# mindspore-lab/mindpose

Hardware: AMD Instinct MI355X
Metric: images/sec at 256x192, HRNet-W32 top-down inference (backbone+head+decode) (higher is better)
Workload: dtype f32; 1 GPU; configs[2]: HRNet-W32 256x192 inference, 1xMI355X per rank, multi-branch conv + fuse layers on fp32 MFMA, HRNetHead, arg-max+shift decode; per_gpu_batch=128, global_batch=128, image=256x192, heatmap=64x48x17, execution_lanes=4

## Files before the change

include/mindpose_hip.h:

```cpp
#ifndef MINDPOSE_HIP_H
#define MINDPOSE_HIP_H

#include <stddef.h>
#include <stdint.h>

#ifdef __cplusplus
extern "C" {
#endif

typedef void* mp_stream_t;

#define MP_OK 0
#define MP_ERR_NULL (-1)
#define MP_ERR_SHAPE (-2)
#define MP_ERR_UNSUPPORTED (-3)
#define MP_ERR_HIP (-4)
#define MP_ERR_WORKSPACE (-5)

const char* mp_version(void);
const char* mp_error_string(int code);
int mp_last_hip_error(void);

#define MP_REFINE_NONE 0
#define MP_REFINE_SHIFT 1
// ... 170 lines not shown
int mp_f16_stem_conv_fwd(const float* x_dev, const float* weight_dev, const float* scale_dev, const float* shift_dev, int relu,
                         void* out_c8_dev, int n, int h, int w, mp_stream_t stream);
int mp_plan_add_stem_conv_f16(mp_plan* plan, const float* x_dev, const float* weight_dev, const float* scale_dev, const float* shift_dev,
                              int relu, void* out_c8_dev, int n, int h, int w);
int mp_f16_expand_reduce_fwd(const void* mid_c8_dev, const void* res_c8_dev, const void* packed_w3_dev, const float* scale3_dev,
                             const float* shift3_dev, int relu3, const void* packed_w1_dev, const float* scale1_dev,
                             const float* shift1_dev, int relu1, void* y_c8_dev, void* z_c8_dev, int n, int cm, int ce, int cr, int h,
                             int w, mp_stream_t stream);
int mp_f16_dual_pw_fwd(const void* x_c8_dev, const void* packed_wa_dev, const float* scale_a_dev, const float* shift_a_dev, int relu_a,
                       const void* packed_wb_dev, const float* scale_b_dev, const float* shift_b_dev, int relu_b, void* ya_c8_dev,
                       void* zb_c8_dev, int n, int cm, int ce, int cr, int h, int w, mp_stream_t stream);
int mp_f16_ds_expand_reduce_fwd(const void* mid_c8_dev, const void* x0_c8_dev, const void* packed_wd_dev, const float* scale_d_dev,
                                const float* shift_d_dev, const void* packed_w3_dev, const float* scale3_dev, const float* shift3_dev,
                                int relu3, const void* packed_w1_dev, const float* scale1_dev, const float* shift1_dev, int relu1,
                                void* y_c8_dev, void* z_c8_dev, int n, int cm, int ce, int cr, int h, int w, mp_stream_t stream);
int mp_plan_add_ds_expand_reduce_f16(mp_plan* plan, const void* mid_c8_dev, const void* x0_c8_dev, const void* packed_wd_dev,
                                     const float* scale_d_dev, const float* shift_d_dev, const void* packed_w3_dev,
                                     const float* scale3_dev, const float* shift3_dev, int relu3, const void* packed_w1_dev,
                                     const float* scale1_dev, const float* shift1_dev, int relu1, void* y_c8_dev, void* z_c8_dev, int n,
                                     int cm, int ce, int cr, int h, int w);
int mp_plan_add_dual_pw_f16(mp_plan* plan, const void* x_c8_dev, const void* packed_wa_dev, const float* scale_a_dev,
                            const float* shift_a_dev, int relu_a, const void* packed_wb_dev, const float* scale_b_dev,
                            const float* shift_b_dev, int relu_b, void* ya_c8_dev, void* zb_c8_dev, int n, int cm, int ce, int cr, int h, int w);
int mp_plan_add_expand_reduce_f16(mp_plan* plan, const void* mid_c8_dev, const void* res_c8_dev, const void* packed_w3_dev,
                                  const float* scale3_dev, const float* shift3_dev, int relu3, const void* packed_w1_dev,
                                  const float* scale1_dev, const float* shift1_dev, int relu1, void* y_c8_dev, void* z_c8_dev, int n,
                                  int cm, int ce, int cr, int h, int w);
int mp_expand_reduce_fwd(const float* mid_dev, const float* res_dev, const float* x0_dev, const float* packed_wd_dev,
                         const float* scale_d_dev, const float* shift_d_dev, const float* packed_w3_dev, const float* scale3_dev,
                         const float* shift3_dev, const float* packed_w1_dev, const float* scale1_dev, const float* shift1_dev,
                         float* y_dev, float* z_dev, int n, int cm, int ce, int cr, int h, int w, mp_stream_t stream);
int mp_plan_add_expand_reduce(mp_plan* plan, const float* mid_dev, const float* res_dev, const float* x0_dev, const float* packed_wd_dev,
                              const float* scale_d_dev, const float* shift_d_dev, const float* packed_w3_dev, const float* scale3_dev,
                              const float* shift3_dev, const float* packed_w1_dev, const float* scale1_dev, const float* shift1_dev,
                              float* y_dev, float* z_dev, int n, int cm, int ce, int cr, int h, int w);
int mp_plan_add_basicblock_f16(mp_plan* plan, const void* x_c8_dev, const void* packed_w1_dev, const float* scale1_dev,
                               const float* shift1_dev, const void* packed_w2_dev, const float* scale2_dev, const float* shift2_dev,
                               void* out_c8_dev, int n, int c, int h, int w, int rows);
int mp_f16_fuse_upsample_sum(const void* base_dev, const void* t1_dev, int s1, const void* t2_dev, int s2, const void* t3_dev,
                             int s3, void* out_dev, int n, int c, int h, int w, int relu, mp_stream_t stream);
int mp_plan_add_conv_f16(mp_plan* plan, const mp_conv_desc* desc, int variant, const void* x_c8_dev, const void* packed_w_dev,
                         const float* scale_dev, const float* shift_dev, const void* res1_c8_dev, const void* res2_c8_dev,
                         void* out_c8_dev);
int mp_plan_add_fuse_sum_f16(mp_plan* plan, const void* base_dev, const void* t1_dev, int s1, const void* t2_dev, int s2,
                             const void* t3_dev, int s3, void* out_dev, int n, int c, int h, int w, int relu);
int mp_plan_add_layout_f16(mp_plan* plan, int to_c8, const void* x_dev, void* out_dev, int n, int c, int h, int w);
int mp_concat_channels(const void* a_dev, int ca, const void* b_dev, int cb, void* out_dev, int n, int h, int w, int c8,
                       mp_stream_t stream);
int mp_plan_add_concat(mp_plan* plan, const void* a_dev, int ca, const void* b_dev, int cb, void* out_dev, int n, int h, int w,
                       int c8);
int mp_col_slice(const void* in_dev, void* out_dev, int rows, int w_in, int start, int w_out, int c8, mp_stream_t stream);
int mp_plan_add_col_slice(mp_plan* plan, const void* in_dev, void* out_dev, int rows, int w_in, int start, int w_out, int c8);
int mp_conv_supported(const mp_conv_desc* desc, int variant);

int mp_warp_affine(const uint8_t* src_dev, const long long* src_offsets_dev, const int* src_hw_dev, const int* flip_dev,
                   const double* trans_dev, void* out_dev, int n, int out_h, int out_w, int normalize, const float mean[3], const float stddev[3],
                   mp_stream_t stream);

int mp_flip_width(const float* in_dev, float* out_dev, int n, int c, int h, int w, mp_stream_t stream);

int mp_resize_pad_normalize(const uint8_t* src_dev, const long long* src_offsets_dev, const int* src_hw_dev, const int* dst_wh_host,
                            float* out_dev, uint8_t* mask_dev, int n, int pad_h, int pad_w, const float mean[3],
                            const float stddev[3], mp_stream_t stream);

int mp_bottomup_train_augment(const uint8_t* src_dev, const long long* src_offsets_dev, const int* src_hw_dev,
                              const uint8_t* mask_src_dev, const long long* mask_offsets_dev, const double* trans_dev,
                              const int* flip_dev, const int* stage_wh_host, float* image_dev, uint8_t* mask_dev, int n, int s,
                              int out_h, int out_w, int hmax, int wmax, const float mean[3], const float stddev[3],
                              mp_stream_t stream);

typedef struct mp_bottomup_stage {
    const float* data_dev;
    int32_t c, h, w;
    int32_t has_tags;
} mp_bottomup_stage;
size_t mp_bottomup_workspace_bytes(int n, int k, int h, int w, int max_num);
int mp_bottomup_parse_nms_topk(const mp_bottomup_stage* stages_host, int num_stages, const uint8_t* mask_dev, int mask_h, int mask_w,
                               int n, int k, int tag_per_joint, int nms_kernel, int max_num, float* heatmap_raw_dev,
                               float* tagging_dev, void* workspace_dev, size_t workspace_bytes, mp_stream_t stream);
int mp_bottomup_gather(const float* heatmap_raw_dev, const float* tagging_dev, const void* workspace_dev, size_t workspace_bytes,
                       int n, int k, int h, int w, int tag_per_joint, int num_tags, int max_num, int shift_coordinate,
                       float* val_k_dev, float* ind_k_dev, float* tag_k_dev, mp_stream_t stream);

int mp_bottomup_refine_missing(const float* heatmap_raw_dev, const float* tagging_dev, const float* mean_tag_dev,
                               const int* person_image_dev, int num_persons, int n, int k, int h, int w, int tag_per_joint,
                               int num_tags, float* found_dev, mp_stream_t stream);

size_t mp_joints_mse_mask_workspace_bytes(int n, int k);
int mp_joints_mse_mask_fwd(const float* pred_dev, long long pred_sn, long long pred_sc, long long pred_sr, const float* target_dev,
                           long long target_sn, long long target_sc, long long target_sr, const void* mask_dev, int mask_is_u8,
                           long long mask_sn, long long mask_sr, float* loss_dev, void* workspace_dev, size_t workspace_bytes, int n,
                           int k, int h, int w, mp_stream_t stream);
int mp_joints_mse_mask_bwd(const float* pred_dev, long long pred_sn, long long pred_sc, long long pred_sr, const float* target_dev,
                           long long target_sn, long long target_sc, long long target_sr, const void* mask_dev, int mask_is_u8,
                           long long mask_sn, long long mask_sr, const float* grad_out_dev, float* grad_pred_dev, long long grad_sn,
                           long long grad_sc, long long grad_sr, int n, int k, int h, int w, mp_stream_t stream);
size_t mp_ae_loss_workspace_bytes(int n);
int mp_ae_loss_fwd(const float* tags_dev, long long tag_batch_stride, const int32_t* tag_ind_dev, float* loss2_dev,
                   void* workspace_dev, size_t workspace_bytes, int n, int m, int k, int hw, mp_stream_t stream);
int mp_ae_loss_bwd(const float* tags_dev, long long tag_batch_stride, const int32_t* tag_ind_dev, const float* grad_out2_dev,
                   float* grad_tags_dev, long long grad_batch_stride, int n, int m, int k, int hw, mp_stream_t stream);
int mp_bottomup_target(const float* keypoints_dev, const int* counts_dev, const int* stage_wh_host, float* target_dev,
                       int32_t* tag_ind_dev, int n, int s, int m, int k, int hmax, int wmax, int max_num, int tag_per_joint,
                       double sigma, mp_stream_t stream);

int mp_f16_bn_train_fwd(const void* z_dev, const float* gamma_dev, const float* beta_dev, const void* res_dev, void* y_dev,
// ... 89 lines not shown
```

mindpose_amd/_lib.py:

```python
import ctypes
import os

import torch

_HERE = os.path.dirname(os.path.abspath(__file__))
LIB_PATH = os.environ.get("MINDPOSE_HIP_LIB", os.path.join(_HERE, "csrc", "libmindpose_hip.so"))

MP_REFINE_NONE, MP_REFINE_SHIFT, MP_REFINE_DARK = 0, 1, 2
MP_CONV_SHARES_CUS = 1
MP_CONV_PHASES4 = 2
MP_ERR_UNSUPPORTED = -3


def env_on(name: str, default: bool = True) -> bool:
    value = os.environ.get(name)
    return value != "0" if default else value == "1"


c_f32p = ctypes.c_void_p
c_int = ctypes.c_int
c_size_t = ctypes.c_size_t
c_i64 = ctypes.c_longlong


# ... 104 lines not shown
    "mp_plan_set_lane": (c_int, [ctypes.c_void_p, c_int]),
    "mp_plan_add_barrier": (c_int, [ctypes.c_void_p]),
    "mp_flip_width": (c_int, [c_f32p, c_f32p] + [c_int] * 4 + [ctypes.c_void_p]),
    "mp_warp_affine": (c_int, [c_f32p] * 6 + [c_int] * 4 + [ctypes.POINTER(ctypes.c_float)] * 2 + [ctypes.c_void_p]),
    "mp_f16_packed_weight_bytes": (c_size_t, [c_int] * 4),
    "mp_f16_activation_bytes": (c_size_t, [c_int] * 4),
    "mp_f16_pack_weight": (c_int, [c_f32p, c_f32p] + [c_int] * 7 + [ctypes.c_void_p]),
    "mp_f16_pack_weight_batch": (c_int, [c_f32p, c_f32p, c_int, ctypes.c_uint, ctypes.c_void_p]),
    "mp_conv_pack_weight_batch": (c_int, [c_f32p, c_f32p, c_int, ctypes.c_uint, ctypes.c_void_p]),
    "mp_f16_to_c8": (c_int, [c_f32p, c_f32p] + [c_int] * 4 + [ctypes.c_void_p]),
    "mp_f16_from_c8": (c_int, [c_f32p, c_f32p] + [c_int] * 4 + [ctypes.c_void_p]),
    "mp_f16_conv2d_fwd": (c_int, [ctypes.POINTER(ConvDesc), c_int] + [c_f32p] * 7 + [ctypes.c_void_p]),
    "mp_f16_conv_stats_parts": (c_int, [ctypes.POINTER(ConvDesc), c_int]),
    "mp_f16_conv2d_fwd_stats": (c_int, [ctypes.POINTER(ConvDesc), c_int] + [c_f32p] * 6 + [ctypes.POINTER(ConvStats), ctypes.c_void_p]),
    "mp_f16_bn_train_fwd_stats": (c_int, [c_f32p] * 9 + [c_int] * 3 + [ctypes.c_float, ctypes.c_float, c_int, c_f32p, c_int, c_f32p,
                                          c_size_t, ctypes.c_void_p]),
    "mp_f16_conv_pre_supported": (c_int, [ctypes.POINTER(ConvDesc), c_int]),
    "mp_f16_conv_supported": (c_int, [ctypes.POINTER(ConvDesc), c_int, c_int, c_int]),
    "mp_f16_bn_train_finalize": (c_int, [c_f32p] * 6 + [c_int] * 3 + [ctypes.c_float, ctypes.c_float, c_f32p, c_int, c_f32p, c_f32p, c_f32p,
                                         c_size_t, ctypes.c_void_p]),
    "mp_f16_bn_train_bwd_stats": (c_int, [c_f32p] * 10 + [c_int] * 3 + [c_f32p, c_int, c_f32p, c_size_t, ctypes.c_void_p]),
    "mp_f16_bn_train_fwd_stats_grouped": (c_int, [ctypes.POINTER(BnFwdJob), c_int, ctypes.c_float, ctypes.c_float, ctypes.c_void_p]),
    "mp_f16_bn_train_bwd_stats_grouped": (c_int, [ctypes.POINTER(BnBwdJob), c_int, ctypes.c_void_p]),
    "mp_f16_ew_stats_parts": (c_int, [c_int] * 3),
    "mp_f16_fuse_term_stats_parts": (c_int, [c_int] * 5),
    "mp_f16_sum_tensors_stats": (c_int, [c_f32p] * 7 + [c_int] * 4 + [c_f32p, c_size_t, ctypes.c_void_p]),
    "mp_f16_fuse_sum_bwd_term_stats": (c_int, [c_f32p] * 3 + [c_int] * 6 + [c_f32p, c_f32p, c_int, c_f32p, c_size_t, ctypes.c_void_p]),
    "mp_optimizer_step": (c_int, [c_int, ctypes.c_void_p, ctypes.c_void_p, ctypes.c_void_p, ctypes.c_void_p, c_size_t, ctypes.c_float,
                                  ctypes.c_float, ctypes.c_float, ctypes.POINTER(ctypes.c_float * 5), ctypes.c_void_p]),
    "mp_f16_basicblock_fwd": (c_int, [c_f32p] * 8 + [c_int] * 5 + [ctypes.c_void_p]),
    "mp_f16_basicblock_supported": (c_int, [c_int] * 4),
    "mp_stem_conv_fwd": (c_int, [c_f32p] * 4 + [c_int, c_f32p] + [c_int] * 3 + [ctypes.c_void_p]),
    "mp_plan_add_stem_conv": (c_int, [ctypes.c_void_p] + [c_f32p] * 4 + [c_int, c_f32p] + [c_int] * 3),
    "mp_f16_stem_conv_fwd": (c_int, [c_f32p] * 4 + [c_int, c_f32p] + [c_int] * 3 + [ctypes.c_void_p]),
    "mp_plan_add_stem_conv_f16": (c_int, [ctypes.c_void_p] + [c_f32p] * 4 + [c_int, c_f32p] + [c_int] * 3),
    "mp_f16_dual_pw_fwd": (c_int, [c_f32p] * 4 + [c_int] + [c_f32p] * 3 + [c_int] + [c_f32p] * 2 + [c_int] * 6 + [ctypes.c_void_p]),
    "mp_plan_add_dual_pw_f16": (c_int, [ctypes.c_void_p] + [c_f32p] * 4 + [c_int] + [c_f32p] * 3 + [c_int] + [c_f32p] * 2 + [c_int] * 6),
    "mp_f16_expand_reduce_fwd": (c_int, [c_f32p] * 5 + [c_int] + [c_f32p] * 3 + [c_int] + [c_f32p] * 2 + [c_int] * 6 + [ctypes.c_void_p]),
    "mp_plan_add_expand_reduce_f16": (c_int, [ctypes.c_void_p] + [c_f32p] * 5 + [c_int] + [c_f32p] * 3 + [c_int] + [c_f32p] * 2 + [c_int] * 6),
    "mp_f16_ds_expand_reduce_fwd": (c_int, [c_f32p] * 8 + [c_int] + [c_f32p] * 3 + [c_int] + [c_f32p] * 2 + [c_int] * 6 + [ctypes.c_void_p]),
    "mp_plan_add_ds_expand_reduce_f16": (c_int, [ctypes.c_void_p] + [c_f32p] * 8 + [c_int] + [c_f32p] * 3 + [c_int] + [c_f32p] * 2 + [c_int] * 6),
    "mp_expand_reduce_fwd": (c_int, [c_f32p] * 14 + [c_int] * 6 + [ctypes.c_void_p]),
    "mp_plan_add_expand_reduce": (c_int, [ctypes.c_void_p] + [c_f32p] * 14 + [c_int] * 6),
    "mp_plan_add_basicblock_f16": (c_int, [ctypes.c_void_p] + [c_f32p] * 8 + [c_int] * 5),
    "mp_f16_fuse_upsample_sum": (c_int, [c_f32p, c_f32p, c_int, c_f32p, c_int, c_f32p, c_int, c_f32p] + [c_int] * 5 + [ctypes.c_void_p]),
    "mp_plan_add_conv_f16": (c_int, [ctypes.c_void_p, ctypes.POINTER(ConvDesc), c_int] + [c_f32p] * 7),
    "mp_plan_add_fuse_sum_f16": (c_int, [ctypes.c_void_p, c_f32p, c_f32p, c_int, c_f32p, c_int, c_f32p, c_int, c_f32p] + [c_int] * 5),
    "mp_plan_add_layout_f16": (c_int, [ctypes.c_void_p, c_int, c_f32p, c_f32p] + [c_int] * 4),
    "mp_concat_channels": (c_int, [c_f32p, c_int, c_f32p, c_int, c_f32p] + [c_int] * 4 + [ctypes.c_void_p]),
    "mp_plan_add_concat": (c_int, [ctypes.c_void_p, c_f32p, c_int, c_f32p, c_int, c_f32p] + [c_int] * 4),
    "mp_col_slice": (c_int, [c_f32p, c_f32p] + [c_int] * 5 + [ctypes.c_void_p]),
    "mp_plan_add_col_slice": (c_int, [ctypes.c_void_p, c_f32p, c_f32p] + [c_int] * 5),
    "mp_conv_supported": (c_int, [ctypes.POINTER(ConvDesc), c_int]),
    "mp_bottomup_workspace_bytes": (c_size_t, [c_int] * 5),
    "mp_bottomup_parse_nms_topk": (c_int, [ctypes.POINTER(BottomUpStage), c_int, c_f32p] + [c_int] * 7 + [c_f32p, c_f32p, c_f32p, c_size_t,
                                                                                                     ctypes.c_void_p]),
    "mp_bottomup_gather": (c_int, [c_f32p, c_f32p, c_f32p, c_size_t] + [c_int] * 8 + [c_f32p, c_f32p, c_f32p, ctypes.c_void_p]),
    "mp_bottomup_refine_missing": (c_int, [c_f32p] * 4 + [c_int] * 7 + [c_f32p, ctypes.c_void_p]),
    "mp_resize_pad_normalize": (c_int, [c_f32p] * 3 + [ctypes.POINTER(ctypes.c_int)] + [c_f32p] * 2 + [c_int] * 3
                                + [ctypes.POINTER(ctypes.c_float)] * 2 + [ctypes.c_void_p]),
    "mp_bottomup_train_augment": (c_int, [c_f32p] * 7 + [ctypes.POINTER(ctypes.c_int)] + [c_f32p] * 2 + [c_int] * 6
                                  + [ctypes.POINTER(ctypes.c_float)] * 2 + [ctypes.c_void_p]),
    "mp_joints_mse_mask_workspace_bytes": (c_size_t, [c_int, c_int]),
    "mp_joints_mse_mask_fwd": (c_int, [c_f32p] + [c_i64] * 3 + [c_f32p] + [c_i64] * 3 + [c_f32p, c_int] + [c_i64] * 2
                               + [c_f32p, c_f32p, c_size_t] + [c_int] * 4 + [ctypes.c_void_p]),
    "mp_joints_mse_mask_bwd": (c_int, [c_f32p] + [c_i64] * 3 + [c_f32p] + [c_i64] * 3 + [c_f32p, c_int] + [c_i64] * 2
                               + [c_f32p, c_f32p] + [c_i64] * 3 + [c_int] * 4 + [ctypes.c_void_p]),
    "mp_ae_loss_workspace_bytes": (c_size_t, [c_int]),
    "mp_ae_loss_fwd": (c_int, [c_f32p, c_i64, c_f32p, c_f32p, c_f32p, c_size_t] + [c_int] * 4 + [ctypes.c_void_p]),
    "mp_ae_loss_bwd": (c_int, [c_f32p, c_i64, c_f32p, c_f32p, c_f32p, c_i64] + [c_int] * 4 + [ctypes.c_void_p]),
    "mp_bottomup_target": (c_int, [c_f32p, c_f32p, ctypes.POINTER(ctypes.c_int), c_f32p, c_f32p] + [c_int] * 8
                           + [ctypes.c_double, ctypes.c_void_p]),
}

EXPORTED_SYMBOLS = tuple(_PROTOTYPES)

_lib = None


def load():
    global _lib
    if _lib is not None:
        return _lib
    if not os.path.exists(LIB_PATH):
        raise MindposeHipError(
            f"{LIB_PATH} not found: the HIP extension is required (no CPU fallback). "
            "Build it with `python -c 'import __graft_entry__ as g; g.build()'` or "
            "`make -C mindpose_amd/csrc -j8`.")
    lib = ctypes.CDLL(LIB_PATH)
    for name, (restype, argtypes) in _PROTOTYPES.items():
        fn = getattr(lib, name)
        fn.restype = restype
        fn.argtypes = argtypes
    _lib = lib
    return lib


def check(rc, what):
    if rc != 0:
        lib = load()
        msg = lib.mp_error_string(rc).decode()
        extra = f" (hipError {lib.mp_last_hip_error()})" if rc == -4 else ""
        raise MindposeHipError(f"{what} failed: {msg}{extra}")


def ptr(t):
# ... 23 lines not shown
```

mindpose_amd/csrc/conv_api.hip:

```cpp
#include <stdlib.h>
#include <string.h>

#include <vector>

#include "conv_f16.h"
#include "conv_mfma.h"
#include "conv_pw.h"
#include "conv_wino.h"
#include "conv_stem.h"
#include "conv_gemm.h"
#include "conv_small.h"
#include "pwchain_f32.h"

namespace mp {

static inline unsigned magic_of(unsigned d) { return d <= 1 ? 0u : (unsigned)(0x100000000ULL / d) + 1u; }
static inline int round_up(int v, int m) { return (v + m - 1) / m * m; }

__device__ __forceinline__ float pack_source(const float* __restrict__ w, int cout, int cin, int kh, int kw, int transposed,
                                             int py, int px, int co, int ci, int t) {
    const int ty = t / kw, tx = t % kw;
    if (transposed == 0) return w[(((size_t)co * cin + ci) * kh + ty) * kw + tx];
    if (transposed == 2) {
        return w[(((size_t)ci * cout + co) * kh + (kh - 1 - ty)) * kw + (kw - 1 - tx)];
// ... 87 lines not shown
    bool gemm;
    GemmLaunch gm;
    bool small_k;
    SmallLaunch sm;
};

constexpr int kGemm = V_COUNT + 2;
constexpr int kSmall = V_COUNT + 3;
constexpr int kPointwise = V_COUNT;

static const int kLdsMax = 150 * 1024;

static int lds_budget() {
    static int v = -1;
    if (v < 0) {
        const char* e = knob("MP_CONV_LDS_KB");
        int kb = e ? atoi(e) : 0;
        v = (kb >= 16 && kb <= 150) ? kb * 1024 : 78 * 1024;
    }
    return v;
}

static int plane_pad(int raw) {
    int v = (raw + 15) / 32 * 32 + 16;
    if (v - 32 >= raw) v -= 32;
    return v;
}

static bool configure(const mp_conv_desc& d, int variant, ConvLaunch& L) {
    int CT, PT;
    variant_dims(variant, CT, PT);
    if (d.kh == 7 && variant != V_CT64_PT192 && variant != V_CT32_PT192_H) return false;
    ConvKParams& p = L.p;
    const int S = d.stride, KS = d.kh;
    p.N = d.n; p.Cin = d.cin; p.H = d.h; p.W = d.w; p.Cout = d.cout;
    p.Cout_pad16 = round_up(d.cout, 16);
    p.Cin_pad4 = round_up(d.cin, 4);
    p.Ho = d.conv_h; p.Wo = d.conv_w; p.pad_t = d.pad_top; p.pad_l = d.pad_left;
    if (p.Wo > PT) return false;
    const int rows_fit = PT / p.Wo;
    if (rows_fit >= p.Ho) {
        p.R = p.Ho;
        p.G = PT / (p.Ho * p.Wo);
        if (p.G > p.N) p.G = p.N;
        if (p.G < 1) p.G = 1;
    } else {
        p.R = rows_fit;
        p.G = 1;
    }
    p.RWo = p.R * p.Wo;
    p.Rin = (p.R - 1) * S + KS;
    p.Wp = (p.Wo - 1) * S + KS;
    if (p.Wp < p.pad_l + p.W && p.pad_l + p.W - p.Wp <= 2) p.Wp = p.pad_l + p.W;
    p.img_plane = p.Rin * p.Wp;
    p.cin_plane = plane_pad(p.G * p.img_plane);
    p.ncols = p.W < p.Wp - p.pad_l ? p.W : p.Wp - p.pad_l;
    if (p.ncols < 1) return false;
    const int T = KS * KS;
    p.vec = ((p.W & 3) == 0 && (p.ncols & 3) == 0) ? 1 : 0;
    p.upr = p.vec ? p.ncols / 4 : p.ncols;
    p.upc = p.G * p.Rin * p.upr;
    const bool light = variant_light(variant) && KS <= 3;
    const int nw = stage_nw(KS, light), ni = stage_ni(KS, light, p.vec != 0);
    const int budget = (light && !knob("MP_CONV_LDS_KB")) ? 52 * 1024 : lds_budget();
    int best_ck = 0;
    for (int ck = 4; ck <= p.Cin_pad4 && ck <= 128; ck += 4) {
        if (p.Cin_pad4 % ck) continue;
        if ((long long)ck * p.upc > (long long)ni * 256) continue;
        if ((long long)ck * T * CT / 4 > (long long)nw * 256) continue;
        const int nbuf = ck < p.Cin_pad4 ? 2 : 1;
        const long long bytes = (long long)nbuf * (ck * p.cin_plane + ck * T * CT) * 4;
        if (bytes > budget && !(ck == 4 && bytes <= kLdsMax)) continue;
        best_ck = ck;
    }
    if (best_ck == 0) return false;
    p.CK = best_ck;
    p.n_chunks = p.Cin_pad4 / p.CK;
    p.nbuf = p.n_chunks > 1 ? 2 : 1;
    p.in_buf = p.CK * p.cin_plane;
    p.w_buf = p.CK * T * CT;
    p.n_ct = (p.Cout_pad16 + CT - 1) / CT;
    p.tiles_y = (p.G > 1 || p.R >= p.Ho) ? 1 : (p.Ho + p.R - 1) / p.R;
    p.tiles_n = (p.N + p.G - 1) / p.G;
    p.out_h = d.out_h; p.out_w = d.out_w; p.out_mul = d.out_mul; p.out_rep = d.out_rep;
    p.off_y = d.out_off_y; p.off_x = d.out_off_x; p.relu = d.relu;
    p.magic_upr = magic_of(p.upr);
    p.magic_upc = magic_of(p.upc);
    p.magic_rin = magic_of(p.Rin);
    p.magic_rwo = magic_of(p.RWo);
    p.magic_wo = magic_of(p.Wo);
    p.total_blocks = p.n_ct * p.tiles_y * p.tiles_n;
    L.ks = KS; L.stride = S; L.variant = variant;
    L.lds_bytes = (size_t)p.nbuf * (p.in_buf + p.w_buf) * 4;
    return L.lds_bytes <= (size_t)kLdsMax;
}

static int choose_variant(const mp_conv_desc& d, ConvLaunch& best, int forced = -1) {
    if (forced == kPointwise) {
        int rc = pw_configure(&d, best.pw);
        if (rc != MP_OK) return rc;
        best.pointwise = true;
        best.ks = 1; best.stride = 1; best.variant = kPointwise;
        best.lds_bytes = best.pw.lds_bytes;
        return MP_OK;
    }
    if (forced == kGemm) {
        int rc = gemm_configure(&d, best.gm);
        if (rc != MP_OK) return rc;
        best.gemm = true;
        best.ks = d.kh; best.stride = best.gm.stride; best.variant = kGemm;
// ... 489 lines not shown
    plan->entries.push_back(e);
    return MP_OK;
}

int mp_plan_add_fuse_sum_f16(mp_plan* plan, const void* base, const void* t1, int s1, const void* t2, int s2, const void* t3,
                             int s3, void* out, int n, int c, int h, int w, int relu) {
    if (!plan || !base || !t1 || !out) return MP_ERR_NULL;
    if (n <= 0 || c <= 0 || h <= 0 || w <= 0) return MP_ERR_SHAPE;
    mp_plan::Entry e{};
    e.kind = 4;
    e.x16 = base; e.out16 = out; e.n = n; e.c = c; e.h = h; e.w = w; e.relu = relu;
    e.t16[0] = t1; e.t16[1] = t2; e.t16[2] = t3; e.s[0] = s1; e.s[1] = s2; e.s[2] = s3;
    e.lane = plan->cur_lane;
    plan->entries.push_back(e);
    return MP_OK;
}

int mp_plan_add_layout_f16(mp_plan* plan, int to_c8, const void* x, void* out, int n, int c, int h, int w) {
    if (!plan || !x || !out) return MP_ERR_NULL;
    if (n <= 0 || c <= 0 || h <= 0 || w <= 0) return MP_ERR_SHAPE;
    mp_plan::Entry e{};
    e.kind = to_c8 ? 5 : 6;
    if (to_c8) { e.x = reinterpret_cast<const float*>(x); e.out16 = out; }
    else { e.x16 = x; e.out = reinterpret_cast<float*>(out); }
    e.n = n; e.c = c; e.h = h; e.w = w;
    e.lane = plan->cur_lane;
    plan->entries.push_back(e);
    return MP_OK;
}

int mp_plan_add_concat(mp_plan* plan, const void* a, int ca, const void* b, int cb, void* out, int n, int h, int w, int c8) {
    if (!plan || !a || !b || !out) return MP_ERR_NULL;
    if (n <= 0 || ca <= 0 || cb <= 0 || h <= 0 || w <= 0) return MP_ERR_SHAPE;
    if (c8 && ca % 8 != 0) return MP_ERR_UNSUPPORTED;
    mp_plan::Entry e{};
    e.kind = 14;
    e.x16 = a; e.t16[0] = b; e.out16 = out;
    e.s[0] = ca; e.s[1] = cb; e.relu = c8 ? 1 : 0;
    e.n = n; e.c = ca + cb; e.h = h; e.w = w;
    e.lane = plan->cur_lane;
    plan->entries.push_back(e);
    return MP_OK;
}

int mp_plan_add_col_slice(mp_plan* plan, const void* in, void* out, int rows, int w_in, int start, int w_out, int c8) {
    if (!plan || !in || !out) return MP_ERR_NULL;
    if (rows <= 0 || w_in <= 0 || w_out <= 0 || start < 0 || start + w_out > w_in) return MP_ERR_SHAPE;
    mp_plan::Entry e{};
    e.kind = 15;
    e.x16 = in; e.out16 = out;
    e.n = rows; e.c = w_in; e.h = start; e.w = w_out; e.relu = c8 ? 1 : 0;
    e.lane = plan->cur_lane;
    plan->entries.push_back(e);
    return MP_OK;
}

int mp_conv_supported(const mp_conv_desc* desc, int variant) {
    if (validate_desc(desc) != MP_OK) return 0;
    ConvLaunch L{};
    return choose_variant(*desc, L, variant) == MP_OK ? 1 : 0;
}

int mp_plan_size(const mp_plan* plan) { return plan ? (int)plan->entries.size() : MP_ERR_NULL; }

int mp_plan_run_range(const mp_plan* plan, int first, int count, mp_stream_t stream) {
    if (!plan) return MP_ERR_NULL;
    if (first < 0 || count < 0 || (size_t)first + count > plan->entries.size()) return MP_ERR_SHAPE;
    for (int i = first; i < first + count; ++i) {
        int rc = run_entry(plan->entries[i], stream);
        if (rc != MP_OK) return rc;
    }
    return MP_OK;
}

int mp_plan_entry_info(const mp_plan* plan, int index, int64_t info[12]) {
    if (!plan || !info) return MP_ERR_NULL;
    if (index < 0 || (size_t)index >= plan->entries.size()) return MP_ERR_SHAPE;
    const mp_plan::Entry& e = plan->entries[index];
    for (int i = 0; i < 12; ++i) info[i] = 0;
    info[0] = e.kind;
    if (e.kind == 0 && e.conv.pointwise) {
        info[1] = 1; info[2] = 1; info[3] = kPointwise; info[4] = e.conv.pw.grid; info[5] = (int64_t)e.conv.pw.lds_bytes;
        info[6] = e.conv.pw.p.Cout; info[7] = 64; info[8] = 64; info[9] = e.conv.pw.cbw; info[10] = e.conv.pw.p.tiles_per_wg;
        info[11] = e.conv.pw.kq;
    } else if (e.kind == 0 && e.conv.gemm) {
        info[1] = e.conv.ks; info[2] = e.conv.gm.stride; info[3] = kGemm; info[11] = e.conv.gm.gather ? 1 : 0; info[4] = (int64_t)e.conv.gm.grid * e.conv.gm.phases; info[5] = (int64_t)e.conv.gm.lds_bytes;
        info[6] = 64 * e.conv.gm.mi; info[7] = 64 * e.conv.gm.ni; info[8] = 16; info[9] = e.conv.gm.phases; info[10] = 1;
    } else if (e.kind == 0 && e.conv.small_k) {
        info[1] = e.conv.ks; info[2] = e.conv.stride; info[3] = e.conv.variant; info[4] = e.conv.sm.grid; info[5] = (int64_t)e.conv.sm.lds_bytes;
        info[6] = 16; info[7] = 16 * e.conv.sm.p.pt; info[8] = e.conv.sm.p.Cin_pad4; info[9] = 1; info[10] = e.conv.sm.p.rows;
    } else if (e.kind == 0) {
        int ct, pt;
        variant_dims(e.conv.variant, ct, pt);
        info[1] = e.conv.ks; info[2] = e.conv.stride; info[3] = e.conv.variant; info[4] = e.conv.p.total_blocks;
        info[5] = (int64_t)e.conv.lds_bytes; info[6] = ct; info[7] = pt; info[8] = e.conv.p.CK; info[9] = e.conv.p.G;
        info[10] = e.conv.p.R;
        info[11] = variant_light(e.conv.variant) ? 1 : 0;
    } else if (e.kind == 3) {
        int ct, pt;
        f16_variant_dims(e.conv16.variant, ct, pt);
        info[1] = e.conv16.ks; info[2] = e.conv16.stride; info[3] = e.conv16.variant; info[4] = e.conv16.p.total_blocks;
        info[5] = (int64_t)e.conv16.lds_bytes; info[6] = ct; info[7] = pt; info[8] = e.conv16.p.PK * 8; info[9] = e.conv16.p.G;
        info[10] = e.conv16.p.R;
        info[11] = f16_variant_light(e.conv16.variant) ? 1 : 0;
    } else if (e.kind == 9) {
        info[1] = 3; info[2] = 1; info[3] = 9 ; info[4] = e.wino.p.total_blocks;
// ... 49 lines not shown
```

mindpose_amd/csrc/conv_mfma.h:

```cpp
#pragma once
#include <type_traits>

#include "common.h"

#ifndef MP_CONV_SCHED
#define MP_CONV_SCHED 1
#endif
#ifndef MP_CONV_STAMPS
#define MP_CONV_STAMPS 0
#endif
#if MP_CONV_STAMPS
#define MP_STAMP(var) unsigned long long var = __builtin_amdgcn_s_memtime(); __builtin_amdgcn_s_waitcnt(0xC07F)
#else
#define MP_STAMP(var) [[maybe_unused]] const unsigned long long var = 0
#endif

namespace mp {

typedef float f32x4 __attribute__((ext_vector_type(4)));
typedef unsigned u32x4 __attribute__((ext_vector_type(4)));

constexpr unsigned kOob = 0x80000000u;
__device__ __forceinline__ __amdgpu_buffer_rsrc_t make_rsrc(const void* base, size_t bytes) {
    return __builtin_amdgcn_make_buffer_rsrc(const_cast<void*>(base), 0, (int)(bytes < 0x7FFFFFF0u ? bytes : 0x7FFFFFF0u), 0x00020000);
}
__device__ __forceinline__ f32x4 buf_load4(__amdgpu_buffer_rsrc_t r, unsigned off) {
    return __builtin_bit_cast(f32x4, __builtin_amdgcn_raw_buffer_load_b128(r, off, 0, 0));
}
__device__ __forceinline__ float buf_load1(__amdgpu_buffer_rsrc_t r, unsigned off) {
    return __builtin_bit_cast(float, __builtin_amdgcn_raw_buffer_load_b32(r, off, 0, 0));
}
__device__ __forceinline__ void buf_store4(__amdgpu_buffer_rsrc_t r, unsigned off, f32x4 v) {
    __builtin_amdgcn_raw_buffer_store_b128(__builtin_bit_cast(u32x4, v), r, off, 0, 0);
}

struct ConvKParams {
    const float* x;
    const float* wp;
    const float* scale;
    const float* shift;
    const float* res1;
    const float* res2;
    float* out;
    int N, Cin, H, W;
    int Cout, Cout_pad16, Cin_pad4;
    int Ho, Wo;
    int pad_t, pad_l;
    int R, G;
    int Rin, Wp;
    int img_plane;
    int cin_plane;
    int CK;
    int n_chunks;
    int n_ct;
    int tiles_y;
    int tiles_n;
    int ncols;
    int vec;
    int upr;
    int upc;
    int in_buf;
    int w_buf;
    int nbuf;
    int out_h, out_w, out_mul, out_rep, off_y, off_x;
    int relu;
    unsigned magic_upr, magic_upc, magic_rin, magic_rwo, magic_wo;
    int RWo;
    int total_blocks;
    unsigned long long* dbg;
};

__device__ __forceinline__ unsigned fastdiv(unsigned e, unsigned d, unsigned magic) {
    return d == 1 ? e : __umulhi(e, magic);
}

template <int KS, int S, int PS, int CS, int WAVES_P, int WAVES_C, int NI, int NW, bool VEC, int OCC>
__global__ __launch_bounds__(256, OCC) void conv_mfma_kernel(const ConvKParams p) {
    static_assert(WAVES_P * WAVES_C == 4, "4 waves per workgroup");
    constexpr int T = KS * KS;
    constexpr int CT = 16 * CS * WAVES_C;
    constexpr int C4 = CT / 4;
    constexpr bool SWZ = (CT % 32) == 0;
    constexpr bool SCHED = MP_CONV_SCHED != 0;
    extern __shared__ __attribute__((aligned(16))) float smem[];
    float* __restrict__ lds_in = smem;
    float* __restrict__ lds_w = smem + p.nbuf * p.in_buf;

    MP_STAMP(t_start);
    [[maybe_unused]] unsigned long long s_load = 0, s_comp = 0, s_store = 0, s_bar = 0;
    const int tid = threadIdx.x, lane = tid & 63, wave = tid >> 6;
    const int wp_i = wave % WAVES_P, wc_i = wave / WAVES_P;
    const int lq = lane >> 4, lr = lane & 15;

    int b = blockIdx.x;
    {
        const int nb = p.total_blocks, q8 = nb >> 3, r8 = nb & 7, xcd = b & 7, j = b >> 3;
        b = (xcd < r8 ? xcd * (q8 + 1) : r8 * (q8 + 1) + (xcd - r8) * q8) + j;
    }
    const int ct = b % p.n_ct;
    b /= p.n_ct;
    const int ty = b % p.tiles_y, tn = b / p.tiles_y;
    const int n0 = tn * p.G, y0 = ty * p.R;
    const int y_in0 = y0 * S - p.pad_t;
    const int HW = p.H * p.W;

    {
        const int n4 = (p.nbuf * p.in_buf) >> 2;
        float4* z = reinterpret_cast<float4*>(lds_in);
        const float4 zero = make_float4(0.f, 0.f, 0.f, 0.f);
        for (int i = tid; i < n4; i += 256) z[i] = zero;
    }

    unsigned isrc[NI];
    int idst[NI];
#pragma unroll
    for (int i = 0; i < NI; ++i) {
        const unsigned u = tid + 256 * i;
        isrc[i] = kOob;
        idst[i] = 0;
        if (u < (unsigned)(p.CK * p.upc)) {
            const unsigned c = fastdiv(u, p.upc, p.magic_upc);
            const unsigned rem = u - c * p.upc;
            const unsigned gr = fastdiv(rem, p.upr, p.magic_upr);
            const unsigned xu = rem - gr * p.upr;
            const unsigned g = p.G > 1 ? fastdiv(gr, p.Rin, p.magic_rin) : 0u;
            const unsigned r = gr - g * p.Rin;
            const int yin = y_in0 + (int)r;
            const unsigned xx = VEC ? xu * 4 : xu;
            if (yin >= 0 && yin < p.H && n0 + (int)g < p.N) {
                isrc[i] = ((g * p.Cin + c) * HW + yin * p.W + xx) * 4u;
                idst[i] = (int)((c << 20) | (c * p.cin_plane + g * p.img_plane + r * p.Wp + p.pad_l + xx));
            }
        }
    }

    int a_off[PS];
#pragma unroll
    for (int ps = 0; ps < PS; ++ps) {
        unsigned pl = (unsigned)((wp_i * PS + ps) * 16 + lr);
        if (pl >= (unsigned)(p.G * p.RWo)) pl = 0;
        const unsigned g = fastdiv(pl, p.RWo, p.magic_rwo);
        const unsigned rem = pl - g * p.RWo;
        const unsigned y = fastdiv(rem, p.Wo, p.magic_wo);
        const unsigned xx = rem - y * p.Wo;
        a_off[ps] = lq * p.cin_plane + g * p.img_plane + (y * S) * p.Wp + xx * S;
    }
    int b_off[CS];
#pragma unroll
    for (int cs = 0; cs < CS; ++cs) {
        int col = (wc_i * CS + cs) * 16 + lr;
        if (SWZ) col ^= (lq & 1) << 4;
        b_off[cs] = lq * CT + col;
    }

    f32x4 acc[PS][CS];
#pragma unroll
    for (int ps = 0; ps < PS; ++ps)
#pragma unroll
        for (int cs = 0; cs < CS; ++cs) acc[ps][cs] = (f32x4){0.f, 0.f, 0.f, 0.f};

    const float* __restrict__ xg = p.x + (size_t)n0 * p.Cin * HW;
    const float* __restrict__ wg = p.wp + ct * CT;
    const int w_rows = (p.CK >> 2) * T * 4;

    using in_t = typename std::conditional<VEC, f32x4, float>::type;
    in_t vin[NI];
    f32x4 vw[NW];
    const int n_img = min(p.G, p.N - n0);
    const __amdgpu_buffer_rsrc_t rs_x = make_rsrc(xg, (size_t)n_img * p.Cin * HW * 4);
    const __amdgpu_buffer_rsrc_t rs_w = make_rsrc(wg, ((size_t)(p.Cin_pad4 >> 2) * T * 4 * p.Cout_pad16 - (size_t)ct * CT) * 4);
    unsigned wsrc[NW];
#pragma unroll
    for (int i = 0; i < NW; ++i) {
        const int u = tid + 256 * i;
        const int row = u / C4, c4 = (u - row * C4) << 2;
        wsrc[i] = (row < w_rows && ct * CT + c4 < p.Cout_pad16) ? (unsigned)(row * p.Cout_pad16 + c4) * 4u : kOob;
    }
    auto stage_load = [&](int ch) {
        const int c0 = ch * p.CK;
        const unsigned xo = (unsigned)c0 * HW * 4u;
#pragma unroll
        for (int i = 0; i < NI; ++i) {
            unsigned off = isrc[i] + xo;
            if (p.Cin & 3) off = (c0 + (idst[i] >> 20) < p.Cin) ? off : kOob;
            if constexpr (VEC) vin[i] = buf_load4(rs_x, off);
            else vin[i] = buf_load1(rs_x, off);
        }
        const unsigned wo = (unsigned)(c0 >> 2) * T * 4u * p.Cout_pad16 * 4u;
#pragma unroll
        for (int i = 0; i < NW; ++i) vw[i] = buf_load4(rs_w, wsrc[i] + wo);
    };
    auto stage_store = [&](int ch, int buf) {
        const int c0 = ch * p.CK;
        float* __restrict__ din = lds_in + buf * p.in_buf;
#pragma unroll
        for (int i = 0; i < NI; ++i) {
            if (isrc[i] != kOob && c0 + (idst[i] >> 20) < p.Cin) {
                float* d = din + (idst[i] & 0xFFFFF);
                if constexpr (VEC) { d[0] = vin[i].x; d[1] = vin[i].y; d[2] = vin[i].z; d[3] = vin[i].w; }
                else d[0] = vin[i];
            }
        }
        float* __restrict__ dw = lds_w + buf * p.w_buf;
#pragma unroll
        for (int i = 0; i < NW; ++i) {
            const int u = tid + 256 * i;
            const int row = u / C4;
            int c4 = (u - row * C4) << 2;
            if (row < w_rows) {
                if (SWZ) c4 ^= (row & 1) << 4;
                *reinterpret_cast<f32x4*>(dw + row * CT + c4) = vw[i];
            }
        }
    };

    stage_load(0);
    __syncthreads();
    stage_store(0, 0);
    __syncthreads();
    MP_STAMP(t_pro);

    const int nq = p.CK >> 2;
    for (int ch = 0; ch < p.n_chunks; ++ch) {
        const int buf = p.nbuf == 2 ? (ch & 1) : 0;
        const bool more = ch + 1 < p.n_chunks;
        MP_STAMP(t0);
        if (more) stage_load(ch + 1);
        MP_STAMP(t1);
        const float* __restrict__ lin = lds_in + buf * p.in_buf;
        const float* __restrict__ lw = lds_w + buf * p.w_buf;
        float av[PS], bv[CS];
#pragma unroll
        for (int ps = 0; ps < PS; ++ps) av[ps] = lin[a_off[ps]];
#pragma unroll
        for (int cs = 0; cs < CS; ++cs) bv[cs] = lw[b_off[cs]];
        if constexpr (KS <= 3) {
            for (int q = 0; q < nq; ++q) {
                const int in_q = q * 4 * p.cin_plane;
                const int w_q = q * T * 4 * CT;
                const int qn = min(q + 1, nq - 1);
    #pragma unroll
                for (int t = 0; t < T; ++t) {
                    const int tn = (t + 1 < T) ? t + 1 : 0;
                    const int in_off = ((t + 1 < T) ? in_q : qn * 4 * p.cin_plane) + (tn / KS) * p.Wp + (tn % KS);
                    const int w_off = ((t + 1 < T) ? w_q : qn * T * 4 * CT) + tn * 4 * CT;
                    float an[PS], bn[CS];
    #pragma unroll
                    for (int ps = 0; ps < PS; ++ps) an[ps] = lin[a_off[ps] + in_off];
    #pragma unroll
                    for (int cs = 0; cs < CS; ++cs) bn[cs] = lw[b_off[cs] + w_off];
    #pragma unroll
                    for (int ps = 0; ps < PS; ++ps)
    #pragma unroll
                        for (int cs = 0; cs < CS; ++cs)
                            acc[ps][cs] = __builtin_amdgcn_mfma_f32_16x16x4f32(av[ps], bv[cs], acc[ps][cs], 0, 0, 0);
                    if (SCHED) {
                        constexpr int NR = PS + CS, NM = PS * CS, NPAIR = NR < NM ? NR : NM;
    #pragma unroll
                        for (int i = 0; i < NPAIR; ++i) {
                            __builtin_amdgcn_sched_group_barrier(0x008, 1, 0);
                            __builtin_amdgcn_sched_group_barrier(0x100, 1, 0);
                        }
                        if (NM > NPAIR) __builtin_amdgcn_sched_group_barrier(0x008, NM - NPAIR, 0);
                        if (NR > NPAIR) __builtin_amdgcn_sched_group_barrier(0x100, NR - NPAIR, 0);
                    }
    #pragma unroll
                    for (int ps = 0; ps < PS; ++ps) av[ps] = an[ps];
    #pragma unroll
                    for (int cs = 0; cs < CS; ++cs) bv[cs] = bn[cs];
                }
            }

        } else {
            for (int q = 0; q < nq; ++q) {
                for (int dy = 0; dy < KS; ++dy) {
#pragma unroll
                    for (int dx = 0; dx < KS; ++dx) {
                        const int in_off = q * 4 * p.cin_plane + dy * p.Wp + dx;
                        const int w_off = (q * T + dy * KS + dx) * 4 * CT;
#pragma unroll
                        for (int ps = 0; ps < PS; ++ps) av[ps] = lin[a_off[ps] + in_off];
#pragma unroll
                        for (int cs = 0; cs < CS; ++cs) bv[cs] = lw[b_off[cs] + w_off];
#pragma unroll
                        for (int ps = 0; ps < PS; ++ps)
#pragma unroll
                            for (int cs = 0; cs < CS; ++cs)
                                acc[ps][cs] = __builtin_amdgcn_mfma_f32_16x16x4f32(av[ps], bv[cs], acc[ps][cs], 0, 0, 0);
                    }
                }
            }
        }
        MP_STAMP(t2);
        if (more) stage_store(ch + 1, buf ^ 1);
        MP_STAMP(t3);
        if (more) __syncthreads();
        MP_STAMP(t4);
// ... 243 lines not shown
```

Measured before the change: 9037 images/s.

## Store stride-2 3x3 conv input rows in even/odd column-split LDS layout

```diff
diff --git a/include/mindpose_hip.h b/include/mindpose_hip.h
--- a/include/mindpose_hip.h
+++ b/include/mindpose_hip.h
@@ -246,6 +246,7 @@
 int mp_col_slice(const void* in_dev, void* out_dev, int rows, int w_in, int start, int w_out, int c8, mp_stream_t stream);
 int mp_plan_add_col_slice(mp_plan* plan, const void* in_dev, void* out_dev, int rows, int w_in, int start, int w_out, int c8);
 int mp_conv_supported(const mp_conv_desc* desc, int variant);
+int mp_conv_geometry(const mp_conv_desc* desc, int variant, int64_t geo[10]);
 
 int mp_warp_affine(const uint8_t* src_dev, const long long* src_offsets_dev, const int* src_hw_dev, const int* flip_dev,
                    const double* trans_dev, void* out_dev, int n, int out_h, int out_w, int normalize, const float mean[3], const float stddev[3],
diff --git a/mindpose_amd/_lib.py b/mindpose_amd/_lib.py
--- a/mindpose_amd/_lib.py
+++ b/mindpose_amd/_lib.py
@@ -180,6 +180,7 @@
     "mp_col_slice": (c_int, [c_f32p, c_f32p] + [c_int] * 5 + [ctypes.c_void_p]),
     "mp_plan_add_col_slice": (c_int, [ctypes.c_void_p, c_f32p, c_f32p] + [c_int] * 5),
     "mp_conv_supported": (c_int, [ctypes.POINTER(ConvDesc), c_int]),
+    "mp_conv_geometry": (c_int, [ctypes.POINTER(ConvDesc), c_int, ctypes.POINTER(ctypes.c_int64)]),
     "mp_bottomup_workspace_bytes": (c_size_t, [c_int] * 5),
     "mp_bottomup_parse_nms_topk": (c_int, [ctypes.POINTER(BottomUpStage), c_int, c_f32p] + [c_int] * 7 + [c_f32p, c_f32p, c_f32p, c_size_t,
                                                                                                      ctypes.c_void_p]),
diff --git a/mindpose_amd/csrc/conv_api.hip b/mindpose_amd/csrc/conv_api.hip
--- a/mindpose_amd/csrc/conv_api.hip
+++ b/mindpose_amd/csrc/conv_api.hip
@@ -163,10 +163,15 @@
     p.Rin = (p.R - 1) * S + KS;
     p.Wp = (p.Wo - 1) * S + KS;
     if (p.Wp < p.pad_l + p.W && p.pad_l + p.W - p.Wp <= 2) p.Wp = p.pad_l + p.W;
+    p.ncols = p.W < p.Wp - p.pad_l ? p.W : p.Wp - p.pad_l;
+    if (p.ncols < 1) return false;
+    p.Wh = 0;
+    if (conv_parity_rows(KS, S)) {
+        p.Wh = (p.Wp + 1) / 2;
+        p.Wp = 2 * p.Wh;
+    }
     p.img_plane = p.Rin * p.Wp;
     p.cin_plane = plane_pad(p.G * p.img_plane);
-    p.ncols = p.W < p.Wp - p.pad_l ? p.W : p.Wp - p.pad_l;
-    if (p.ncols < 1) return false;
     const int T = KS * KS;
     p.vec = ((p.W & 3) == 0 && (p.ncols & 3) == 0) ? 1 : 0;
     p.upr = p.vec ? p.ncols / 4 : p.ncols;
@@ -762,6 +767,20 @@
     e.n = rows; e.c = w_in; e.h = start; e.w = w_out; e.relu = c8 ? 1 : 0;
     e.lane = plan->cur_lane;
     plan->entries.push_back(e);
+    return MP_OK;
+}
+
+int mp_conv_geometry(const mp_conv_desc* desc, int variant, int64_t geo[10]) {
+    if (!geo) return MP_ERR_NULL;
+    int rc = validate_desc(desc);
+    if (rc != MP_OK) return rc;
+    if (variant < 0 || variant >= V_COUNT) return MP_ERR_UNSUPPORTED;
+    ConvLaunch L{};
+    if (!configure(*desc, variant, L)) return MP_ERR_UNSUPPORTED;
+    const bool light = variant_light(variant) && desc->kh <= 3;
+    geo[0] = L.p.Wp; geo[1] = L.p.Wh; geo[2] = L.p.Rin; geo[3] = L.p.img_plane; geo[4] = L.p.cin_plane; geo[5] = L.p.G;
+    geo[6] = L.p.CK; geo[7] = L.p.n_chunks; geo[8] = (int64_t)L.lds_bytes;
+    geo[9] = L.p.CK == 4 ? kLdsMax : (light && !knob("MP_CONV_LDS_KB")) ? 52 * 1024 : lds_budget();
     return MP_OK;
 }
 
diff --git a/mindpose_amd/csrc/conv_mfma.h b/mindpose_amd/csrc/conv_mfma.h
--- a/mindpose_amd/csrc/conv_mfma.h
+++ b/mindpose_amd/csrc/conv_mfma.h
@@ -48,6 +48,7 @@
     int pad_t, pad_l;
     int R, G;
     int Rin, Wp;
+    int Wh;
     int img_plane;
     int cin_plane;
     int CK;
@@ -70,6 +71,8 @@
     unsigned long long* dbg;
 };
 
+constexpr bool conv_parity_rows(int ks, int stride) { return ks == 3 && stride == 2; }
+
 __device__ __forceinline__ unsigned fastdiv(unsigned e, unsigned d, unsigned magic) {
     return d == 1 ? e : __umulhi(e, magic);
 }
@@ -82,6 +85,7 @@
     constexpr int C4 = CT / 4;
     constexpr bool SWZ = (CT % 32) == 0;
     constexpr bool SCHED = MP_CONV_SCHED != 0;
+    constexpr bool PAR = conv_parity_rows(KS, S);
     extern __shared__ __attribute__((aligned(16))) float smem[];
     float* __restrict__ lds_in = smem;
     float* __restrict__ lds_w = smem + p.nbuf * p.in_buf;
@@ -129,7 +133,9 @@
             const unsigned xx = VEC ? xu * 4 : xu;
             if (yin >= 0 && yin < p.H && n0 + (int)g < p.N) {
                 isrc[i] = ((g * p.Cin + c) * HW + yin * p.W + xx) * 4u;
-                idst[i] = (int)((c << 20) | (c * p.cin_plane + g * p.img_plane + r * p.Wp + p.pad_l + xx));
+                const unsigned col = p.pad_l + xx;
+                const unsigned in_row = PAR ? (col & 1) * p.Wh + (col >> 1) : col;
+                idst[i] = (int)((c << 20) | (c * p.cin_plane + g * p.img_plane + r * p.Wp + in_row));
             }
         }
     }
@@ -143,7 +149,7 @@
         const unsigned rem = pl - g * p.RWo;
         const unsigned y = fastdiv(rem, p.Wo, p.magic_wo);
         const unsigned xx = rem - y * p.Wo;
-        a_off[ps] = lq * p.cin_plane + g * p.img_plane + (y * S) * p.Wp + xx * S;
+        a_off[ps] = lq * p.cin_plane + g * p.img_plane + (y * S) * p.Wp + (PAR ? xx : xx * S);
     }
     int b_off[CS];
 #pragma unroll
@@ -190,6 +196,7 @@
 #pragma unroll
         for (int i = 0; i < NW; ++i) vw[i] = buf_load4(rs_w, wsrc[i] + wo);
     };
+    const int par_step = (p.pad_l & 1) ? 1 - p.Wh : p.Wh;
     auto stage_store = [&](int ch, int buf) {
         const int c0 = ch * p.CK;
         float* __restrict__ din = lds_in + buf * p.in_buf;
@@ -197,7 +204,10 @@
         for (int i = 0; i < NI; ++i) {
             if (isrc[i] != kOob && c0 + (idst[i] >> 20) < p.Cin) {
                 float* d = din + (idst[i] & 0xFFFFF);
-                if constexpr (VEC) { d[0] = vin[i].x; d[1] = vin[i].y; d[2] = vin[i].z; d[3] = vin[i].w; }
+                if constexpr (VEC && PAR) {
+                    float* e = d + par_step;
+                    d[0] = vin[i].x; d[1] = vin[i].z; e[0] = vin[i].y; e[1] = vin[i].w;
+                } else if constexpr (VEC) { d[0] = vin[i].x; d[1] = vin[i].y; d[2] = vin[i].z; d[3] = vin[i].w; }
                 else d[0] = vin[i];
             }
         }
@@ -242,7 +252,8 @@
     #pragma unroll
                 for (int t = 0; t < T; ++t) {
                     const int tn = (t + 1 < T) ? t + 1 : 0;
-                    const int in_off = ((t + 1 < T) ? in_q : qn * 4 * p.cin_plane) + (tn / KS) * p.Wp + (tn % KS);
+                    const int in_off = ((t + 1 < T) ? in_q : qn * 4 * p.cin_plane) + (tn / KS) * p.Wp +
+                                       (PAR ? ((tn % KS) & 1) * p.Wh + ((tn % KS) >> 1) : (tn % KS));
                     const int w_off = ((t + 1 < T) ? w_q : qn * T * 4 * CT) + tn * 4 * CT;
                     float an[PS], bn[CS];
     #pragma unroll
```

Result: no change. 8995 images/s (-0.5%).
